# dselivanov/rsparse

Hardware: AMD Instinct MI355X
Metric: als_iterations_per_sec (higher is better)
Workload: dtype f32 (Gram products of rows > 512 / <= 32 non-zeros as 2 x fp16 / 3 x bf16 split terms of the fp32 operands, fp32 accumulate; everything else fp32); 1 GPU; WRMF implicit ALS, CG(3), synthetic 10000000x1000000, 500155883 nnz, rank 128, lambda 0.1; survey_config=3, feedback=implicit, n_items=1000000, nnz=500155883, rank=128, solver=conjugate_gradient, cg_steps=3, parallelism=rows sharded x1, factors replicated

## Files before the change

rsparse_amd/csrc/wrmf_capi.cpp:

```cpp
#include "../../include/rsparse_wrmf_hip.h"

#include <cxxabi.h>

#include <algorithm>
#include <cfloat>
#include <cmath>
#include <cstdio>
#include <cstdlib>
#include <cstring>
#include <string>
#include <vector>

#include "wrmf_capi_common.h"
#include "wrmf_topk_plan.h"

using namespace rsparse_hip;

struct rsparse_hip_csc {
  DevCSC d;
  int device = 0;
  std::vector<void*> owned;
};

namespace {
// ... 180 lines not shown
  return implicit || solver != RSPARSE_SOLVER_CHOLESKY || lambda != 0.0;
}

int check_variant(unsigned solver, int with_biases, double global_bias, bool implicit = true) {
  if (solver > RSPARSE_SOLVER_NNLS) return fail(RSPARSE_HIP_ERR_INVALID, "unknown solver code");
  if (with_biases && implicit && solver == RSPARSE_SOLVER_CONJUGATE_GRADIENT)
    return fail(RSPARSE_HIP_ERR_UNSUPPORTED, "with_user_item_bias + conjugate_gradient with implicit feedback is not on the device path");
  (void)global_bias;
  return RSPARSE_HIP_OK;
}

struct BiasTerms {
  const float* rhs_vals;
  const float* loss_tgt;
  const float* rhs_init;
  float tgt_const = 1.f;
  float gbias = 0.f;
};

hipError_t take_value_stats(const DevCSC& d, const float* d_X, int64_t nx, hipStream_t s, const float* d_absmax) {
  if (d.vals_frozen && !d.vstats && hipMalloc(&d.vstats, 2 * sizeof(unsigned)) != hipSuccess) d.vstats = nullptr;
  if (d.vals_frozen && d.vstats && d.vstats_valid && d.vstats_stream == s)
    return launch_ne_stats(d_X, nx, d.vals, d.nnz, g_ws.ne_stats, s, d_absmax, d.vstats, nullptr);
  hipError_t e = launch_ne_stats(d_X, nx, d.vals, d.nnz, g_ws.ne_stats, s, d_absmax, nullptr,
                                 (d.vals_frozen && d.vstats) ? d.vstats : nullptr);
  if (e == hipSuccess && d.vals_frozen && d.vstats) { d.vstats_valid = true; d.vstats_stream = s; }
  return e;
}

int run_half_iteration(const rsparse_hip_csc* conf, bool implicit, const float* d_X, float* d_Y,
                       const float* d_XtX, int rank, double lambda, unsigned solver, unsigned cg_steps,
                       int dynamic_lambda, double* d_loss_rows_out, hipStream_t s, const BiasTerms* bias = nullptr,
                       const float* d_absmax = nullptr) {
  if (!conf) return fail(RSPARSE_HIP_ERR_INVALID, "conf is NULL");
  if (!d_X || !d_Y) return fail(RSPARSE_HIP_ERR_INVALID, "X or Y is NULL");
  if (implicit && !d_XtX) return fail(RSPARSE_HIP_ERR_INVALID, "XtX is NULL");
  if (rank <= 0) return fail(RSPARSE_HIP_ERR_INVALID, "rank must be positive");
  if (rank > RSPARSE_HIP_MAX_RANK) return fail(RSPARSE_HIP_ERR_UNSUPPORTED, "rank > 256 is not on the device path");
  int rc = check_variant(solver, 0, 0.0);
  if (rc) return rc;
  if ((rc = g_ws.ensure_device())) return rc;
  const DevCSC& d = conf->d;
  const bool pad_to_128 = solver == RSPARSE_SOLVER_CHOLESKY && !bias && rank > 64 && rank < 128 && zero_padding_is_neutral(implicit, solver, lambda);
  const bool pad_to_64 = solver == RSPARSE_SOLVER_CHOLESKY && !bias && rank < 64 && zero_padding_is_neutral(implicit, solver, lambda);
  if (((rank % 4 != 0 && rank < 128) || pad_to_128 || pad_to_64) && zero_padding_is_neutral(implicit, solver, lambda)) {
    const int kp = pad_to_128 ? 128 : (pad_to_64 ? 64 : ((rank + 3) & ~3));
    const size_t nx = (size_t)d.n_rows * kp, ny = (size_t)d.n_cols * kp, ng = (size_t)kp * kp;
    HIP_TRY(g_ws.pad_buf.ensure(nx + ny + ng + 256 + 16));
    float* Xp = g_ws.pad_buf;
// ... 140 lines not shown
    if (implicit) {
      a.ne_stats = g_ws.ne_stats;
      a.mf_XtX = d_XtX;
      if (rank != 128) {
        HIP_TRY(g_ws.mf_G.ensure((size_t)128 * 128));
        hipError_t pe = launch_pad_gramian(d_XtX, rank, 128, g_ws.mf_G, s);
        if (pe != hipSuccess) return hip_fail(pe, "launch_pad_gramian");
        a.mf_XtX = g_ws.mf_G;
      }
    }
  }
  if (!a.ne_stats && (cgq || ne_chol) && implicit && (qs.ne.wg > 0 || qs.mf_n > 0) && ne_supported(rank) && (!bias || gb_cg)) {
    if ((rc = want_stats())) return rc;
    a.ne_stats = g_ws.ne_stats;
    if (gb_cg && cgq) {
      const int n_ne = d.q_off[1];
      HIP_TRY(g_ws.gb_r0.ensure((size_t)n_ne * rank));
      HIP_TRY(g_ws.gb_slot.ensure((size_t)d.n_cols));
      hipError_t ge = launch_gb_row_terms(a, d.q_order, n_ne, g_ws.gb_r0, g_ws.gb_slot, s);
      if (ge != hipSuccess) return hip_fail(ge, "launch_gb_row_terms");
      a.ne_r0 = g_ws.gb_r0; a.ne_r0_slot = g_ws.gb_slot;
    }
  }
  if (cgq && !ne_supported(rank) && d.q_stream_off && d.q_nnz[0] > 0 && cg_steps >= 1 && cg_steps <= 4) {
    HIP_TRY(g_ws.tscr.ensure((size_t)(cg_steps + 1) * (size_t)d.q_nnz[0]));
    a.tscr = g_ws.tscr;
  }
  if (!cg && solver == RSPARSE_SOLVER_CHOLESKY && d.q_order && d.q_n_lr > 0 && chol_lr_supported(a, implicit)) {
    HIP_TRY(g_ws.lr_M.ensure((size_t)3 * 128 * 128));
    if ((rc = want_stats())) return rc;
    a.lr_rows = d.q_order + d.q_lr_first; a.n_lr = d.q_n_lr; a.lr_flags = g_ws.ne_stats + 2; a.lr_M = g_ws.lr_M;
    a.lr_n_gt32 = d.q_gt32 - d.q_lr_first; a.lr_n_gt16 = d.q_pair_first - d.q_lr_first;
    a.lr_n_gt48 = d.q_gt48 - d.q_lr_first;
  }
  const bool chol = !cg && solver == RSPARSE_SOLVER_CHOLESKY;
  if (chol && d.q_order && d.q_n_lr > 0 && chol_lrx_supported(a, implicit)) {
    if ((rc = want_stats())) return rc;
    a.wave_stats = g_ws.ne_stats;
    a.lr_rows = d.q_order + d.q_lr_first; a.n_lr = d.q_n_lr; a.lrx = 1;
    a.lr_n_gt32 = d.q_gt32 - d.q_lr_first; a.lr_n_gt16 = d.q_pair_first - d.q_lr_first;
    a.lr_n_gt48 = d.q_gt48 - d.q_lr_first;
  }
  if (chol && chol_wave_supported(rank) && padded_rank(rank) == 64) {
    if ((rc = want_stats())) return rc;
    a.wave_stats = g_ws.ne_stats;
  }
// ... 42 lines not shown
  if (rank < 2) return fail(RSPARSE_HIP_ERR_INVALID, "with_biases needs rank >= 2 (a row of ones and a bias row)");
  if (rank > RSPARSE_HIP_MAX_RANK) return fail(RSPARSE_HIP_ERR_UNSUPPORTED, "rank > 256 is not on the device path");
  int rc = g_ws.ensure_device();
  if (rc) return rc;
  const DevCSC& d = conf->d;
  const int k1 = rank - 1;
  const int xoff = is_x_bias_last_row ? 0 : 1;
  const int xb = is_x_bias_last_row ? rank - 1 : 0;
  const int ioff = is_x_bias_last_row ? 1 : 0;
  const int ooff = is_x_bias_last_row ? 0 : 1;
  const int k1p = zero_padding_is_neutral(false, solver, lambda) ? std::min((k1 + 3) & ~3, RSPARSE_HIP_MAX_RANK) : k1;
  const size_t nx = (size_t)d.n_rows * k1p, ny = (size_t)d.n_cols * k1p, nv = (size_t)std::max<int64_t>(d.nnz, 1);
  HIP_TRY(g_ws.bias_buf.ensure(nx + ny + nv + 16));
  float* Xp = g_ws.bias_buf;
  float* Yp = Xp + nx;
  float* vp = Yp + ny;
  hipError_t e;
  if ((e = launch_pad_rows(d_X, rank, xoff, k1, k1p, d.n_rows, Xp, s)) != hipSuccess) return hip_fail(e, "launch_pad_rows");
  if ((e = launch_pad_rows(d_Y, rank, ioff, k1, k1p, d.n_cols, Yp, s)) != hipSuccess) return hip_fail(e, "launch_pad_rows");
  e = launch_bias_shift_values(d.vals, d.row_idx, d_X, rank, xb, d.nnz, vp, s);
  if (e != hipSuccess) return hip_fail(e, "launch_bias_shift_values");
  rsparse_hip_csc shifted;
  shifted.d = conf->d; shifted.device = conf->device;
  shifted.d.vals_frozen = false; shifted.d.vstats_valid = false; shifted.d.vstats = nullptr;
  shifted.d.vals = vp;
  rc = run_half_iteration(&shifted, false, Xp, Yp, nullptr, k1p, lambda, solver, cg_steps, dynamic_lambda,
                          d_loss_rows_out, s);
  if (rc) return rc;
  if (d.n_cols > 0)
    HIP_TRY(hipMemcpy2DAsync(d_Y + ooff, (size_t)rank * 4, Yp, (size_t)k1p * 4, (size_t)k1 * 4, (size_t)d.n_cols,
                             hipMemcpyDeviceToDevice, s));
  return RSPARSE_HIP_OK;
}

int run_half_iteration_implicit_biased(const rsparse_hip_csc* conf, const float* d_X, float* d_Y, const float* d_XtX,
                                       int rank, double lambda, unsigned solver, int is_x_bias_last_row,
                                       double* d_loss_rows_out, hipStream_t s, double global_bias = 0.0,
                                       bool dbl_threshold = false) {
  if (!conf) return fail(RSPARSE_HIP_ERR_INVALID, "conf is NULL");
  if (!d_X || !d_Y || !d_XtX) return fail(RSPARSE_HIP_ERR_INVALID, "X, Y or XtX is NULL");
  if (rank < 2) return fail(RSPARSE_HIP_ERR_INVALID, "with_biases needs rank >= 2 (a row of ones and a bias row)");
  if (rank > RSPARSE_HIP_MAX_RANK) return fail(RSPARSE_HIP_ERR_UNSUPPORTED, "rank > 256 is not on the device path");
  int rc = g_ws.ensure_device();
  if (rc) return rc;
  const DevCSC& d = conf->d;
  const int k1 = rank - 1;
  const int xoff = is_x_bias_last_row ? 0 : 1, xb = is_x_bias_last_row ? rank - 1 : 0;
// ... 219 lines not shown
}

int rsparse_hip_values_to_float_device(int64_t n, const double* d_src, float* d_dst, void* stream) {
  if (n < 0) return fail(RSPARSE_HIP_ERR_INVALID, "negative length");
  if (n > 0 && (!d_src || !d_dst)) return fail(RSPARSE_HIP_ERR_INVALID, "NULL array");
  if (n == 0) return RSPARSE_HIP_OK;
  hipError_t e = launch_f64_to_f32(d_src, d_dst, (size_t)n, static_cast<hipStream_t>(stream));
  if (e != hipSuccess) return hip_fail(e, "launch_f64_to_f32");
  return RSPARSE_HIP_OK;
}

int rsparse_hip_csc_destroy(rsparse_hip_csc* m) {
  if (!m) return RSPARSE_HIP_OK;
  for (void* p : m->owned) (void)hipFree(p);
  if (m->d.vstats) (void)hipFree(m->d.vstats);
  delete m;
  return RSPARSE_HIP_OK;
}

int rsparse_hip_csc_freeze_values(rsparse_hip_csc* m, int frozen) {
  if (!m) return fail(RSPARSE_HIP_ERR_INVALID, "NULL handle");
  m->d.vals_frozen = frozen != 0;
  m->d.vstats_valid = false;
  return RSPARSE_HIP_OK;
}

int rsparse_hip_csc_info(const rsparse_hip_csc* m, int64_t info_out[40]) {
  if (!m || !info_out) return fail(RSPARSE_HIP_ERR_INVALID, "NULL argument");
  for (int b = 0; b < 40; b++) info_out[b] = 0;
  for (int b = 0; b < 6; b++) {
    info_out[8 + b] = m->d.q_off[b + 1] - m->d.q_off[b];
    info_out[14 + b] = m->d.q_nnz[b];
  }
  info_out[20] = m->d.q_cfg;
  info_out[21] = m->d.q_ne.nseg;
  for (int b = 0; b < 6; b++) {
    info_out[22 + b] = cgq_bucket_wpr(m->d.q_cfg, b);
    info_out[28 + b] = cgq_bucket_capq(m->d.q_cfg, b);
    info_out[34 + b] = cgq_bucket_waves(m->d.q_cfg, b) * (cgq_bucket_stream(m->d.q_cfg, b) ? -1 : 1);
  }
  info_out[0] = m->d.n_rows; info_out[1] = m->d.n_cols; info_out[2] = m->d.nnz;
  info_out[3] = m->d.n_long; info_out[4] = m->d.max_len; info_out[5] = m->d.nnz_long;
  info_out[6] = m->d.n_empty; info_out[7] = m->d.short_max;
  return RSPARSE_HIP_OK;
}

// ... 909 lines not shown
```

rsparse_amd/csrc/wrmf_cg_mf.hip:

```cpp
#include <cstdio>
#include <utility>

#pragma clang diagnostic ignored "-Winline-asm"

#include "wrmf_internal.h"
#include "wrmf_device.h"

namespace rsparse_hip {
namespace {
using namespace dev;
constexpr int MF_A0 = 0;
#define MF_TOP "a255"
}
}

#include "wrmf_mf.h"

namespace rsparse_hip {
namespace {

__device__ __forceinline__ void cgm_operands_hi(const float (&x)[16], f16x8& h0, f16x8& h1) {
  float b0[8], b1[8];
#pragma unroll
  for (int e = 0; e < 8; e++) {
// ... 471 lines not shown
      for (int I = 0; I < 4; I++) {
        b[I] = sw.rhs[32 * I + n];
        x[I] = sw.x0[4 * n + I];
      }
    }
    auto rd_m1 = [&](auto tt, auto vt) { return mf_rd<16 * decltype(tt)::value + decltype(vt)::value>(); };
    auto g_tile = [&](auto tt, float (&g)[16]) {
      constexpr int T = decltype(tt)::value;
#pragma unroll
      for (int q = 0; q < 4; q++) {
        const float4 t = sm.G[T][ln][q];
        g[4 * q] = t.x; g[4 * q + 1] = t.y; g[4 * q + 2] = t.z; g[4 * q + 3] = t.w;
      }
    };
    float r[4], p[4], ap[4];
    cgm_matvec(rd_m1, g_tile, sw, un_m1, n, hf, ln, x, ap);
#pragma unroll
    for (int I = 0; I < 4; I++) { r[I] = b[I] - ap[I]; p[I] = r[I]; }
    double rsold = (double)cgm_dot(r, r, hf);
    for (int stp = 0; stp < a.cg_steps; stp++) {
      cgm_matvec(rd_m1, g_tile, sw, un_m1, n, hf, ln, p, ap);
      const float alpha = (float)(rsold / (double)cgm_dot(p, ap, hf));
#pragma unroll
      for (int I = 0; I < 4; I++) { x[I] = fmaf(alpha, p[I], x[I]); r[I] = fmaf(-alpha, ap[I], r[I]); }
      const double rsnew = (double)cgm_dot(r, r, hf);
      if (rsnew < (double)kCgTol) break;
      const float beta = (float)(rsnew / rsold);
#pragma unroll
      for (int I = 0; I < 4; I++) p[I] = fmaf(p[I], beta, r[I]);
      rsold = rsnew;
    }
    if (hf == 0) {
      int row2 = row;
      asm volatile("" : "+s"(row2));
      float* yr = a.Y + (size_t)row2 * k;
      *reinterpret_cast<float4*>(yr + 4 * n) = make_float4(x[0], x[1], x[2], x[3]);
    }
    auto rd_m2 = [&](auto tt, auto vt) {
      constexpr int T = decltype(tt)::value, v = decltype(vt)::value;
      if constexpr (T < 6) return mf_rd<160 + 16 * T + v>();
      else return hi[T - 6][v];
    };
    float yMy;
    {
      wave_sync();
      if (hf == 0) {
#pragma unroll
// ... 30 lines not shown
    wave_sync();
  }
  if (lane == 0) a.loss_partials[loss_slot0 + 4 * blockIdx.x + wv] = sw.loss;
}

}
}

#define CGM_KERNEL(NAME, SYM)                                                                                                     \
  extern "C" __global__ __launch_bounds__(256, 1) __attribute__((amdgpu_num_vgpr(128))) void NAME(                                  \
      rsparse_hip::AlsArgs a, const int32_t* __restrict__ rows, int n_rows, int loss_slot0) {                                       \
    rsparse_hip::als_cg_mf_body<SYM>(a, rows, n_rows, loss_slot0);                                                                  \
  }
CGM_KERNEL(rsparse_hip_als_cg_mf_implicit, true)
CGM_KERNEL(rsparse_hip_als_cg_mf_implicit_any, false)
#undef CGM_KERNEL

namespace rsparse_hip {

bool cg_mf_supported(int k, bool implicit) { return implicit && k == 128; }
int cg_mf_grid(int n_rows) { return std::max(1, std::min((n_rows + 3) / 4, kCgMfGrid)); }
int cg_mf_loss_slots(int n_rows) { return 2 * 4 * cg_mf_grid(n_rows); }

hipError_t launch_als_cg_mf(const AlsArgs& a, const int32_t* rows, int n_rows, int loss_slot0, hipStream_t s, hipEvent_t* ev_slot) {
  if (n_rows <= 0) return hipSuccess;
  if (!a.ne_stats || !cg_mf_supported(a.k, true) || (reinterpret_cast<uintptr_t>(a.X) & 3)) return hipErrorInvalidValue;
  const int grid = cg_mf_grid(n_rows);
  auto kern = rsparse_hip_als_cg_mf_implicit;
  auto kern2 = rsparse_hip_als_cg_mf_implicit_any;
  const int b1 = (int)sizeof(CgmSmem<12>), b2 = (int)sizeof(CgmSmem<20>);
  hipError_t e;
  if ((e = hipFuncSetAttribute(reinterpret_cast<const void*>(kern), hipFuncAttributeMaxDynamicSharedMemorySize, b1)) != hipSuccess) return e;
  if ((e = hipFuncSetAttribute(reinterpret_cast<const void*>(kern2), hipFuncAttributeMaxDynamicSharedMemorySize, b2)) != hipSuccess) return e;
  prof_note(ev_slot, reinterpret_cast<const void*>(kern));
  hipLaunchKernelGGL(kern, dim3(grid), dim3(256), b1, s, a, rows, n_rows, loss_slot0);
  hipLaunchKernelGGL(kern2, dim3(grid), dim3(256), b2, s, a, rows, n_rows, loss_slot0 + 4 * grid);
  return hipGetLastError();
}

}
```

rsparse_amd/csrc/wrmf_cgp.hip:

```cpp
#include "wrmf_internal.h"
#include "wrmf_device.h"

namespace rsparse_hip {
namespace {

using namespace dev;

constexpr int kPairMaxSweeps = 4;

template <int NQ, bool QUAD = false>
struct PairSmem {
  static constexpr int KP = 128, ps = KP + 8, os = QUAD ? KP + 8 : KP + 4;
  static constexpr int cols = QUAD ? 16 : 8;
  static constexpr int pcs = QUAD ? 2 * ps : ps;
  static constexpr size_t gfrag = NQ == 16 ? (size_t)4 * 16 * 1024 : 0;
  static constexpr size_t nxt = NQ == 16 ? (size_t)4 * 2 * 2 * 64 * 4 : 0;
  static constexpr size_t pub = (size_t)2 * cols * ps * 2, out = (size_t)cols * os * 4;
  static_assert(!QUAD || (pub == out && (size_t)pcs * 2 == (size_t)os * 4), "QUAD: one column, one stretch of LDS");
  static constexpr size_t bytes = gfrag + (QUAD ? pub : pub + out) + (size_t)4 * 8 * NQ * 4 + nxt + 16;
};
static_assert(PairSmem<16>::bytes <= 81920 && PairSmem<16, true>::bytes <= 81920, "two workgroups per CU");

template <bool GB, bool KFULL = false, int NQ = 8, bool QUAD = false>
__global__ __launch_bounds__(256, 2) void als_cgp_kernel(AlsArgs a, const int32_t* __restrict__ rows, int n_rows, int iters,
// ... 387 lines not shown
    auto dot16 = [&](const float(&u)[RPN], const float(&w)[RPN]) {
      float s = 0.f;
#pragma unroll
      for (int rr = 0; rr < RPN; rr++) s = fmaf(u[rr], w[rr], s);
      return row16_sum(s);
    };

    float dummy = 0.f;
    sweep(x, 0, r, dummy);
    if constexpr (KFULL)
      request_indices(it + 1 < iters && ridx(it + 1) < n_rows, p1_c, p2_c - p1_c, (it + 1) & 1);
#pragma unroll
    for (int rr = 0; rr < RPN; rr++) p[rr] = r[rr];
    float rsold = dot16(r, r);
    bool conv = !live;
    for (int itc = 0; itc < a.cg_steps; ++itc) {
      sweep(p, 1, ap, dummy);
      const float pap = dot16(p, ap);
      const float alpha = conv ? 0.f : (float)((double)rsold / (double)pap);
      wave_sync();
      if (lgrp) tacc[lslot] = fmaf(alpha, tcur[lslot], tacc[lslot]);
      wave_sync();
#pragma unroll
      for (int rr = 0; rr < RPN; rr++) {
        x[rr] = fmaf(alpha, p[rr], x[rr]);
        r[rr] = fmaf(-alpha, ap[rr], r[rr]);
      }
      const float rsnew = dot16(r, r);
      if (!conv) {
        if (rsnew < kCgTol) {
          conv = true;
        } else {
          const float beta = (float)((double)rsnew / (double)rsold);
#pragma unroll
          for (int rr = 0; rr < RPN; rr++) p[rr] = fmaf(p[rr], beta, r[rr]);
          rsold = rsnew;
        }
      }
    }
    float rl = 0.f;
    sweep(x, 2, ap, rl);
    if constexpr (KFULL) {
      settle_indices();
    }
    if (live) {
      const float xx = dot16(x, x);
      wloss += (double)rl + a.lambda_loss * (double)xx;
      if (QUAD || g2 == 0) {
#pragma unroll
        for (int b = 0; b < NV; b++) {
          const int off = b * 16 * VW + i * VW;
          if (off < k) {
            float4 pc;
            float* pf = reinterpret_cast<float*>(&pc);
#pragma unroll
            for (int c = 0; c < VW; c++) pf[c] = x[b * VW + c];
            *reinterpret_cast<float4*>(yrow + off) = pc;
          }
        }
// ... 49 lines not shown
```

rsparse_amd/csrc/wrmf_cgq.hip:

```cpp
#include <algorithm>

#include "wrmf_internal.h"
#include "wrmf_device.h"

namespace rsparse_hip {
namespace {

using namespace dev;

constexpr int kGvFirstMinCapq = 16;
constexpr int kStreamPrefixQ = 4;
constexpr int kIdxPrefetchMaxWpr = 2;

constexpr int kMaxSavedSweeps = 4;

template <int KP>
struct QG {
  static constexpr int RPN = KP / 16;
  static constexpr int VW = RPN >= 4 ? 4 : RPN;
  static constexpr int NV = RPN / VW;
  __device__ static __forceinline__ int elem(int i, int r) { return (r / VW) * (16 * VW) + i * VW + (r % VW); }
};

template <int VW>
// ... 796 lines not shown
          if (s2 == itc) alph[s2] = alpha;
        if constexpr (TSAVE) {
          wave_sync();
          const int ln = opaque_lane<WIDEQ>(lane);
#pragma unroll
          for (int s2 = 0; s2 < NSL; s2++) {
            const int sl = NSL == 1 ? (lane & (CAP - 1)) : ln + 64 * s2;
            if (CAP % 64 == 0 || sl < CAP) tacc[sl] = fmaf(alpha, tcur[sl], tacc[sl]);
          }
          wave_sync();
        }
        if constexpr (CVLDS) {
          if (g == 0) {
#pragma unroll
            for (int b = 0; b < NV; b++) {
              piece_t pc = *x_piece(b);
              float* pf = reinterpret_cast<float*>(&pc);
#pragma unroll
              for (int c = 0; c < VW; c++) pf[c] = fmaf(alpha, p[b * VW + c], pf[c]);
              *x_piece(b) = pc;
            }
          }
        }
#pragma unroll
        for (int rr = 0; rr < RPN; rr++) {
          if constexpr (!CVLDS) x[rr] = fmaf(alpha, p[rr], x[rr]);
          r[rr] = fmaf(-alpha, ap[rr], r[rr]);
        }
        const float rsnew = dot16(r, r);
        if (rsnew < kCgTol) {
          conv = true;
        } else {
          const float beta = (float)((double)rsnew / (double)rsold);
#pragma unroll
          for (int rr = 0; rr < RPN; rr++) p[rr] = fmaf(p[rr], beta, r[rr]);
          rsold = rsnew;
        }
      }
    }
    if constexpr (CVLDS) {
      wave_sync();
#pragma unroll
      for (int b = 0; b < NV; b++) {
        const piece_t pc = *x_piece(b);
        const float* pf = reinterpret_cast<const float*>(&pc);
#pragma unroll
        for (int c = 0; c < VW; c++) x[b * VW + c] = pf[c];
      }
    }
    float rl = 0.f;
    sweep(x, 2, ap, rl, live);
    if constexpr (META_LATE) p1_c = rfl(p1_c), p2_c = rfl(p2_c);
    if constexpr (DMAPF) wait_vm<0>();
    if constexpr (IDXPF && STREAM == 0) {
      asm volatile("" : "+v"(pf_id), "+v"(pf_c));
    }
    if (live && tw == 0) {
      const float xx = dot16(x, x);
      const double wl_row = IMPLICIT ? (double)rl + a.lambda_loss * (double)xx : (double)(rl + lam_use * xx);
// ... 135 lines not shown
            forked = true;                                                                                  \
          }                                                                                                 \
          bs = g_bs.st[B];                                                                                  \
          if ((err = hipStreamWaitEvent(bs, g_bs.fork, 0)) != hipSuccess) return err;                       \
        }                                                                                                   \
        if (D.stream && ne_supported(a.k)) {                                                                \
           \
           \
           \
           \
          const bool mside = overlap && q.ne.wg > 0 && q.mf_n > 0;                                          \
           \
          if (mside && (err = hipEventRecord(g_bs.fork0, s)) != hipSuccess) return err;                     \
          if (q.ne.wg > 0 &&                                                                                \
              (err = launch_als_ne(a, q, IMPLICIT, a.loss_partials + slot, bs, q.mf_n > 0 ? nullptr : (ev ? ev + B : nullptr))) != hipSuccess) \
            return err;                                                                                     \
          if (q.mf_n > 0) {                                                                                 \
            hipStream_t ms = bs;                                                                            \
            if (mside) {                                                                                    \
              ms = g_bs.st[B];                                                                              \
              if ((err = hipStreamWaitEvent(ms, g_bs.fork0, 0)) != hipSuccess) return err;                  \
            }                                                                                               \
            if ((err = launch_als_cg_mf(a, q.mf_rows, q.mf_n, (int)(slot + (size_t)(q.ne.entries + q.ne.nsplit)), ms, \
                                        ev ? ev + B : nullptr)) != hipSuccess)                              \
              return err;                                                                                   \
            if (mside) {                                                                                    \
              if ((err = hipEventRecord(g_bs.done[B], ms)) != hipSuccess) return err;                       \
              if ((err = hipStreamWaitEvent(s, g_bs.done[B], 0)) != hipSuccess) return err;                 \
            }                                                                                               \
          }                                                                                                 \
        } else if constexpr (D.stream && KP > 32) {        \
          return hipErrorInvalidValue;                                                                      \
        } else if constexpr (B == 1 && team4_split(KP, GB)) {                                              \
           \
           \
          const int first = q.off[B], wide = team4_wide_first(q), split = team4_first(q);                   \
          const int n_main = wide - first, n_w4 = split - wide, n_t4 = q.off[B + 1] - split;                \
          const int g_main = cgq_bucket_grid(n_main, B, CFG), g_w4 = cgq_team4_wide_grid(n_w4);             \
          if ((err = launch_bucket<KP, D.waves, D.capq, D.wpr, D.stream, IMPLICIT, GB>(a, q.order + first, n_main, g_main, slot, \
                                                                                  bs, ev ? ev + B : nullptr)) != hipSuccess) \
            return err;                                                                                     \
          if ((err = launch_bucket<KP, kTeam4Waves, kTeam4WideCapq, kTeam4Waves, 0, IMPLICIT, GB>(          \
                   a, q.order + wide, n_w4, g_w4, slot + (size_t)g_main * D.waves, bs,                      \
                   n_main > 0 ? nullptr : (ev ? ev + B : nullptr))) != hipSuccess)                          \
            return err;                                                                                     \
          if ((err = launch_bucket<KP, kTeam4Waves, kTeam4Capq, kTeam4Waves, 0, IMPLICIT, GB>(              \
                   a, q.order + split, n_t4, cgq_team4_grid(n_t4),                                          \
// ... 109 lines not shown
```

rsparse_amd/csrc/wrmf_internal.h:

```cpp
#pragma once
#include <hip/hip_runtime.h>
#include <cstdint>
#include <string>

#include "wrmf_schedule.h"

namespace rsparse_hip {

constexpr float kCgTol = 1e-10f;
constexpr double kCgTolD = 1e-10;
constexpr int kScdMaxIter = 10000;
constexpr float kScdTol = 1e-4f;
constexpr double kScdTolD = 1e-4;
constexpr float kNnlsEps = 1e-16f;
constexpr double kNnlsEpsD = 1e-16;

struct NeListSet {
  const int32_t* rows = nullptr;
  const int32_t* ptr = nullptr;
  int wg = 0;
  int entries = 0;
  const int32_t* segs = nullptr;
  int nseg = 0;
  const int32_t* split_rows = nullptr;
// ... 13 lines not shown
  int max_len = 0;
  const int32_t* q_order = nullptr;
  int q_off[7] = {0, 0, 0, 0, 0, 0, 0};
  int q_cfg = 0;
  int q_pair_first = 0;
  int q_team4_first = 0;
  int q_team4_wide_first = 0;
  int64_t q_nnz[6] = {0, 0, 0, 0, 0, 0};
  const int64_t* q_stream_off = nullptr;
  int q_n_chol_long = 0;
  int q_gt32 = 0;
  int q_gt48 = 0;
  int q_lr_first = 0, q_n_lr = 0;
  NeListSet q_ne;
  NeListSet q_ne1;
  int q_n_nec = 0;
  NeListSet q_nec;
  int64_t nnz_long = 0;
  int n_empty = 0;
  mutable bool vals_frozen = false;
  mutable bool vstats_valid = false;
  mutable unsigned* vstats = nullptr;
  mutable hipStream_t vstats_stream = nullptr;
};

struct AlsArgs {
  const int32_t* col_ptrs;
  const int32_t* row_idx;
  const float* vals;
  const float* X;
  float* Y;
  const float* XtX;
  const int32_t* long_rows;
  int n_long;
  int n_cols;
  int k;
  int cg_steps;
  float lambda;
  double lambda_loss;
  int dynamic_lambda;
  double* loss_partials;
  int* fail_counter;
  int* fail_rows;
  int fail_cap;
  const float* zero_row;
  const float* rhs_vals;
// ... 21 lines not shown
  float* lr_M;
  const int32_t* ne_segs;
  float* ne_seg_scratch;
  int* ne_seg_flags;
  int ne_chol;
  int ne_chol_min;
  const unsigned* ne_stats;
  const float* mf_XtX;
  const unsigned* wave_stats;
};

struct QSchedule {
  const int32_t* order;
  int off[7];
  int pair_first;
  int team4_first;
  int team4_wide_first;
  bool pair_wide;
  bool pair_quad = false;
  int cfg;
  NeListSet ne;
  const int32_t* mf_rows = nullptr;
  int mf_n = 0;
};
int cgq_default_cfg();
void cgq_set_launch_mode(int mode);
int cgq_num_buckets();
int cgq_bucket_wpr(int cfg, int b);
int cgq_bucket_capq(int cfg, int b);
int cgq_bucket_waves(int cfg, int b);
int cgq_bucket_stream(int cfg, int b);
int cgq_bucket_grid(int n_rows, int bucket, int cfg);
int cgq_team4_grid(int n_rows);
int cgq_team4_wide_grid(int n_rows);
int cgq_bucket_of(int len, int cfg);
size_t cgq_loss_slots(const QSchedule& q, int k, bool implicit);
bool cgp_supported(int k, bool implicit);
bool cgp_wide_supported(int k, bool implicit, bool gbias);
bool cgp_quad_supported(int k, bool implicit, bool gbias);
enum CgpForm { kCgpPair = 0, kCgpWide = 1, kCgpQuad = 2 };
inline int cgp_rows_per_wave(CgpForm form) { return form == kCgpQuad ? 4 : 2; }
hipError_t launch_als_cgp(const AlsArgs& a, const int32_t* rows, int n_rows, CgpForm form, size_t loss_slot0, hipStream_t s,
                          hipEvent_t* ev_slot);
bool ne_supported(int k);
constexpr int kNeMinLen = 512;
constexpr int kNeSegFloats = 4 * (11 * 16 * 64 + 128 + 2);
// ... 18 lines not shown
constexpr int kCholLongGrid = 512;
constexpr int kCholLrGrid = 65536;
size_t chol2_loss_slots(int n_cols);
bool chol_lr_supported(const AlsArgs& a, bool implicit);
bool chol_lrx_supported(const AlsArgs& a, bool implicit);
hipError_t launch_als_chol_lrx(const AlsArgs& a, const int32_t* rows, int n_rows, const unsigned* stats, int loss_slot0,
                               hipStream_t s, hipEvent_t* ev_slot);
hipError_t launch_als_chol_lr(const AlsArgs& a, const int32_t* rows, int n_rows, float* M, float* Mt, unsigned* flags,
                              int loss_slot0, hipStream_t s, hipEvent_t* ev_slot = nullptr);
hipError_t launch_als_chol2(const AlsArgs& a, bool implicit, hipStream_t s, hipEvent_t* ev = nullptr);
bool chol_wave_supported(int k);
hipError_t launch_als_chol_wave(const AlsArgs& a, bool implicit, int grid, int loss_slot0, hipStream_t s, hipEvent_t* ev_slot);
constexpr int kCholMfMax = 512;
constexpr int kCholMfGrid = 256 * 32;
bool chol_mf_supported(int k);
int chol_mf_grid(int n_rows);
int chol_mf_loss_slots(int n_rows, bool implicit);
hipError_t launch_als_chol_mf(const AlsArgs& a, bool implicit, const int32_t* rows, int n_rows, int loss_slot0, hipStream_t s,
                              hipEvent_t* ev_slot);
constexpr int kCgMfGrid = 256 * 16;
bool cg_mf_supported(int k, bool implicit);
int cg_mf_grid(int n_rows);
int cg_mf_loss_slots(int n_rows);
hipError_t launch_als_cg_mf(const AlsArgs& a, const int32_t* rows, int n_rows, int loss_slot0, hipStream_t s, hipEvent_t* ev_slot);
hipError_t launch_als_nnls(const AlsArgs& a, bool implicit, hipStream_t s, hipEvent_t* ev = nullptr);
constexpr int kLuGrid = 64;
constexpr int kFailCap = 1 << 16;
hipError_t launch_als_lu_fallback(const AlsArgs& a, bool implicit, size_t loss_slot0, hipStream_t s);
hipError_t launch_fail_roll(int* fails, hipStream_t s);
constexpr int kSumStageBlocks = 256;
hipError_t launch_sum_partials(const double* partials, size_t n, double* out, hipStream_t s, double* tail = nullptr);
hipError_t launch_bias_shift_values(const float* vals, const int32_t* row_idx, const float* X, int k, int bias_row,
                                    int64_t nnz, float* out, hipStream_t s);
hipError_t launch_bias_sweep(const int32_t* p, const int32_t* i, const float* x, const float* other, int n_cols,
                             float lambda, int dynamic_lambda, int non_negative, float* out, hipStream_t s);
hipError_t launch_values_sum(const float* x, int64_t n, double* partials, double* out, hipStream_t s);
hipError_t launch_bias_implicit_terms(const float* vals, const int32_t* row_idx, const float* X, int k, int bias_row,
                                      int64_t nnz, float global_bias, float* rhs_vals, float* loss_tgt, hipStream_t s);
hipError_t launch_bias_rhs_init(const float* X, int k, int off, int k1, int bias_row, float global_bias, int n,
                                float* scratch, float* out, hipStream_t s);
size_t bias_rhs_init_scratch_floats();
hipError_t launch_pad_rows(const float* src, int src_stride, int src_off, int k1, int k1p, int64_t n, float* dst, hipStream_t s);
hipError_t launch_pad_gramian(const float* G, int k1, int k1p, float* Gp, hipStream_t s);
hipError_t launch_bias_implicit_prep(const int32_t* p, const float* x, int n_cols, int n_other, double lambda,
                                     double* means, double* adj, hipStream_t s);
hipError_t launch_bias_implicit_sweep(const int32_t* p, const int32_t* i, const float* x, const float* other, int n_cols,
                                      int n_other, const double* other_sum, const double* means, const double* adj,
// ... 239 lines not shown
```

rsparse_amd/csrc/wrmf_kernels.hip:

```cpp
#include "wrmf_internal.h"
#include "wrmf_device.h"

namespace rsparse_hip {
namespace {

using namespace dev;

template <int KP, int T, int W, bool IMPLICIT>
struct CgSmem {
  static constexpr int LDT = Geo<KP>::LDT;
  static constexpr size_t gram_floats = IMPLICIT ? (size_t)KP * KP : 0;
  static constexpr size_t tile_floats = (size_t)W * T * LDT;
  static constexpr size_t vec_floats = (size_t)W * KP;
  static constexpr size_t red_floats = (size_t)2 * W * KP + 2 * W;
  static constexpr size_t short_bytes = (gram_floats + tile_floats + vec_floats) * 4 + 16;
  static constexpr size_t long_bytes = (gram_floats + tile_floats + vec_floats + red_floats) * 4 + 16;
};

template <int KP, int W>
__device__ __forceinline__ void load_gram_lds(float* sG, const float* __restrict__ G, int k, int tid) {
  for (int e = tid; e < KP * KP; e += W * 64) {
    const int r = e / KP, c = e % KP;
    sG[e] = (r < k && c < k) ? G[(size_t)r * k + c] : 0.f;
  }
// ... 75 lines not shown
    for (int u = 0; u < EPL; u++) { p[u] = r[u]; rs = fmaf(r[u], r[u], rs); }
    float rsold = wave_sum(rs);

    for (int it = 0; it < a.cg_steps; ++it) {
      wave_sync();
      put_vec<KP>(vec, p, lane, active);
      wave_sync();
      t = tile_dot<KP, T>(tile, vec, lane);
      wgt = jvalid ? (IMPLICIT ? (c - 1.f) * t : t) : 0.f;
#pragma unroll
      for (int u = 0; u < EPL; u++) ap[u] = 0.f;
      tile_axpy<KP>(tile, wgt, cnt, lane, active, ap);
      if constexpr (IMPLICIT) {
        gram_mv<KP>(sG, vec, 0, KP, lane, active, 1.f, ap);
      } else {
#pragma unroll
        for (int u = 0; u < EPL; u++) ap[u] = fmaf(lam_use, p[u], ap[u]);
      }
      float pap = 0.f;
#pragma unroll
      for (int u = 0; u < EPL; u++) pap = fmaf(p[u], ap[u], pap);
      pap = wave_sum(pap);
      const float alpha = (float)((double)rsold / (double)pap);
      rs = 0.f;
#pragma unroll
      for (int u = 0; u < EPL; u++) {
        x[u] = fmaf(alpha, p[u], x[u]);
        r[u] = fmaf(-alpha, ap[u], r[u]);
        rs = fmaf(r[u], r[u], rs);
      }
      const float rsnew = wave_sum(rs);
      if (rsnew < kCgTol) break;
      const float beta = (float)((double)rsnew / (double)rsold);
#pragma unroll
      for (int u = 0; u < EPL; u++) p[u] = fmaf(p[u], beta, r[u]);
      rsold = rsnew;
    }

    wave_sync();
    put_vec<KP>(vec, x, lane, active);
    wave_sync();
    t = tile_dot<KP, T>(tile, vec, lane);
    const float d = IMPLICIT ? ltgt - t : c - t;
    const float lj = (jvalid && lane < T) ? (IMPLICIT ? c * d * d : d * d) : 0.f;
    const float rl = wave_sum(lj);
    float xx = 0.f;
#pragma unroll
    for (int u = 0; u < EPL; u++) xx = fmaf(x[u], x[u], xx);
    xx = wave_sum(xx);
    wloss += IMPLICIT ? (double)rl + a.lambda_loss * (double)xx : (double)(rl + lam_use * xx);
// ... 123 lines not shown
#pragma unroll
          for (int u = 0; u < EPL; u++) out[u] = fmaf(mode == 0 ? -lam_use : lam_use, v[u], out[u]);
        } else if (gb && mode == 0) {
#pragma unroll
          for (int u = 0; u < EPL; u++) out[u] += (active && e0 + u < k) ? a.rhs_init[e0 + u] : 0.f;
        }
      }
      buf ^= 1;
    };

    float dummy = 0.f;
    sweep(x, 0, r, dummy);
    float rs = 0.f;
#pragma unroll
    for (int u = 0; u < EPL; u++) { p[u] = r[u]; rs = fmaf(r[u], r[u], rs); }
    float rsold = wave_sum(rs);
    for (int it = 0; it < a.cg_steps; ++it) {
      sweep(p, 1, ap, dummy);
      float pap = 0.f;
#pragma unroll
      for (int u = 0; u < EPL; u++) pap = fmaf(p[u], ap[u], pap);
      pap = wave_sum(pap);
      const float alpha = (float)((double)rsold / (double)pap);
      rs = 0.f;
#pragma unroll
      for (int u = 0; u < EPL; u++) {
        x[u] = fmaf(alpha, p[u], x[u]);
        r[u] = fmaf(-alpha, ap[u], r[u]);
        rs = fmaf(r[u], r[u], rs);
      }
      const float rsnew = wave_sum(rs);
      if (rsnew < kCgTol) break;
      const float beta = (float)((double)rsnew / (double)rsold);
#pragma unroll
      for (int u = 0; u < EPL; u++) p[u] = fmaf(p[u], beta, r[u]);
      rsold = rsnew;
    }
    float rl = 0.f;
    sweep(x, 2, ap, rl);
    float xx = 0.f;
#pragma unroll
    for (int u = 0; u < EPL; u++) xx = fmaf(x[u], x[u], xx);
    xx = wave_sum(xx);
    if (wv == 0) {
      wloss += IMPLICIT ? (double)rl + a.lambda_loss * (double)xx : (double)(rl + lam_use * xx);
#pragma unroll
      for (int u = 0; u < EPL; u++)
        if (active && e0 + u < k) yrow[e0 + u] = x[u];
    }
  }
// ... 316 lines not shown
```

rsparse_amd/csrc/wrmf_ne.hip:

```cpp
#include <type_traits>
#include <utility>

#include "wrmf_internal.h"
#include "wrmf_device.h"
#include "wrmf_ldlt.h"

namespace rsparse_hip {
namespace {

using namespace dev;

constexpr int kStepNnz = 16;

struct NeMfmaOp { int slot, m, R, C, pa, pb; };
struct NeUnit { int kind, t, pair; };

template <int KP, int NS, bool IMPLICIT, bool SYM = false, bool QUAD = false>
struct NeRoles {
  static_assert(!SYM || (IMPLICIT && NS == 2), "SYM: implicit feedback, two fp16 terms");
  static_assert(!QUAD || (SYM && KP == 128), "QUAD: the fp16 path at rank 128");
  static constexpr int NB = KP / 32;
  static constexpr int NT = NB * (NB + 1) / 2;
  static constexpr bool PAIR = IMPLICIT && KP == 128 && !QUAD;
  static constexpr int NROLES = QUAD ? 4 : (PAIR ? 2 : 1);
// ... 930 lines not shown
    } else {
    float r[NB], p[NB], ap[NB];
#pragma unroll
    for (int t = 0; t < NB; t++) p[t] = x[t];
    float r0x[NB];
#pragma unroll
    for (int t = 0; t < NB; t++) r0x[t] = 0.f;
    if constexpr (GB) {
      const int sl = sload(a.ne_r0_slot + row);
#pragma unroll
      for (int t = 0; t < NB; t++) r0x[t] = (32 * t + d < k) ? a.ne_r0[(size_t)sl * k + 32 * t + d] : 0.f;
    }
    double rsold = 0.0;
    bool conv = false;
    for (int it = 0; it <= a.cg_steps; ++it) {
      matvec(p, ap);
      if (it == 0) {
#pragma unroll
        for (int t = 0; t < NB; t++) p[t] = r[t] = (b[t] - ap[t]) + r0x[t];
        rsold = (double)dot(r, r);
      } else if (!conv) {
        const float alpha = (float)(rsold / (double)dot(p, ap));
#pragma unroll
        for (int t = 0; t < NB; t++) {
          x[t] = fmaf(alpha, p[t], x[t]);
          r[t] = fmaf(-alpha, ap[t], r[t]);
        }
        const double rsnew = (double)dot(r, r);
        if (rsnew < (double)kCgTol) {
          conv = true;
        } else {
          const float beta = (float)(rsnew / rsold);
#pragma unroll
          for (int t = 0; t < NB; t++) p[t] = fmaf(p[t], beta, r[t]);
          rsold = rsnew;
        }
      }
    }
    }

    wave_sync();
    if (h == 0) {
#pragma unroll
      for (int t = 0; t < NB; t++) pub[32 * t + d] = x[t];
    }
    wave_sync();
    float qf = 0.f;
    with_role([&](auto rc) { qf = quad_form(rc, pub, x); });
    if (lane == 0) sScal[16 + wv] = qf;
    const float yb = dot(x, b), yy = dot(x, x);
    __syncthreads();
    if (wv == 0) {
      const double q = ((double)sScal[16] + (double)sScal[17]) + ((double)sScal[18] + (double)sScal[19]);
      const double tau = GB ? (double)a.loss_tgt_const : 1.0;
      const double fit = tau * tau * sc_row - 2.0 * tau * (double)yb + q;
      const double reg = IMPLICIT ? a.lambda_loss * (double)yy : (double)(lam_use * yy);
      if (lane == 0) {
        sYloss[nbuf] = row_bad ? 0.0 : fit + reg;
// ... 215 lines not shown
```

rsparse_amd/csrc/wrmf_wide_cg.hip:

```cpp
#include <algorithm>

#include "wrmf_internal.h"
#include "wrmf_device.h"

namespace rsparse_hip {
namespace {

using namespace dev;

template <int EPL>
struct WVec {
  float c[EPL];
};

struct WideCgArgs {
  const int32_t* col_ptrs;
  const int32_t* row_idx;
  const float* vals;
  const float* X;
  float* Y;
  const float* XtX;
  int n_cols, k, cg_steps, dynamic_lambda, n_hi;
  double lambda_loss;
  double* loss_partials;
// ... 150 lines not shown
    const float lam_use = IMPLICIT ? (float)a.lambda_loss : (float)(a.lambda_loss * (a.dynamic_lambda ? (double)n : 1.0));
    Vec x, r, pv;
#pragma unroll
    for (int e = 0; e < EPL; e++) x.c[e] = lk[e] ? yrow[lane + 64 * e] : 0.f;
    {
      const Vec t0 = wide_row_pass<EPL, IMPLICIT, 0, TEAM>(a, k, p1, n, x, lk, lc, lane, wv, sT);
      Vec g0;
      if constexpr (IMPLICIT) g0 = gmv(x);
#pragma unroll
      for (int e = 0; e < EPL; e++) r.c[e] = t0.c[e] - (IMPLICIT ? g0.c[e] : lam_use * x.c[e]);
    }
    pv = r;
    double rsold = (double)dot(r, r);
    for (int it = 0; it < a.cg_steps; it++) {
      Vec ap = wide_row_pass<EPL, IMPLICIT, 1, TEAM>(a, k, p1, n, pv, lk, lc, lane, wv, sT);
      {
        Vec g1;
        if constexpr (IMPLICIT) g1 = gmv(pv);
#pragma unroll
        for (int e = 0; e < EPL; e++) ap.c[e] += IMPLICIT ? g1.c[e] : lam_use * pv.c[e];
      }
      const float alpha = (float)(rsold / (double)dot(pv, ap));
#pragma unroll
      for (int e = 0; e < EPL; e++) {
        x.c[e] = fmaf(alpha, pv.c[e], x.c[e]);
        r.c[e] = fmaf(-alpha, ap.c[e], r.c[e]);
      }
      const double rsnew = (double)dot(r, r);
      if (rsnew < (double)kCgTol) break;
      const float beta = (float)(rsnew / rsold);
#pragma unroll
      for (int e = 0; e < EPL; e++) pv.c[e] = fmaf(pv.c[e], beta, r.c[e]);
      rsold = rsnew;
    }
    if (TEAM == 1 || wv == 0) {
#pragma unroll
      for (int e = 0; e < EPL; e++)
        if (lane + 64 * e < k) yrow[lane + 64 * e] = x.c[e];
    }
    const Vec lrow = wide_row_pass<EPL, IMPLICIT, 2, TEAM>(a, k, p1, n, x, lk, lc, lane, wv, sT);
    const float xx = dot(x, x);
    wloss += IMPLICIT ? (double)lrow.c[0] + a.lambda_loss * (double)xx : (double)(lrow.c[0] + lam_use * xx);
  }
  if constexpr (TEAM > 1) {
    if (tid == 0) a.loss_partials[slot0 + blockIdx.x] = wloss;
  } else {
    if (lane == 0) sLoss[wv] = wloss;
    __syncthreads();
    if (tid == 0) a.loss_partials[slot0 + blockIdx.x] = (sLoss[0] + sLoss[1]) + (sLoss[2] + sLoss[3]);
  }
// ... 49 lines not shown
```

Baseline: 8.819 iterations/s.

## Skip final CG residual update and launch only the live cg_mf kernel variant

Across the CG kernels, the last iteration now stops after updating x and skips the residual update, its norm and the p update, since nothing uses them afterwards. Some template variants are excluded via constexpr flags. Separately, after value stats are computed for frozen values, one stats word is read back to the host once. That flag selects which of the two cg_mf kernels is needed, and the unneeded one is skipped with its loss slots zeroed. The trade is a one-time host sync when stats are taken, plus added branching in the kernels.

After: 8.835 iterations/s, median of 5. No clear change (+0.2%).

```diff
diff --git a/rsparse_amd/csrc/wrmf_capi.cpp b/rsparse_amd/csrc/wrmf_capi.cpp
--- a/rsparse_amd/csrc/wrmf_capi.cpp
+++ b/rsparse_amd/csrc/wrmf_capi.cpp
@@ -226,9 +226,16 @@
   if (d.vals_frozen && !d.vstats && hipMalloc(&d.vstats, 2 * sizeof(unsigned)) != hipSuccess) d.vstats = nullptr;
   if (d.vals_frozen && d.vstats && d.vstats_valid && d.vstats_stream == s)
     return launch_ne_stats(d_X, nx, d.vals, d.nnz, g_ws.ne_stats, s, d_absmax, d.vstats, nullptr);
+  d.vstats_valid = false; d.vstats_lt1 = -1;
   hipError_t e = launch_ne_stats(d_X, nx, d.vals, d.nnz, g_ws.ne_stats, s, d_absmax, nullptr,
                                  (d.vals_frozen && d.vstats) ? d.vstats : nullptr);
-  if (e == hipSuccess && d.vals_frozen && d.vstats) { d.vstats_valid = true; d.vstats_stream = s; }
+  if (e == hipSuccess && d.vals_frozen && d.vstats) {
+    unsigned lt1 = 0;
+    if ((e = hipMemcpyAsync(&lt1, d.vstats + 1, sizeof(unsigned), hipMemcpyDeviceToHost, s)) != hipSuccess) return e;
+    if ((e = hipStreamSynchronize(s)) != hipSuccess) return e;
+    d.vstats_lt1 = lt1 != 0u ? 1 : 0;
+    d.vstats_valid = true; d.vstats_stream = s;
+  }
   return e;
 }
 
@@ -415,6 +422,7 @@
       a.ne_r0 = g_ws.gb_r0; a.ne_r0_slot = g_ws.gb_slot;
     }
   }
+  if (qs.mf_n > 0 && stats_taken && d.vals_frozen && d.vstats_valid) qs.mf_live = d.vstats_lt1;
   if (cgq && !ne_supported(rank) && d.q_stream_off && d.q_nnz[0] > 0 && cg_steps >= 1 && cg_steps <= 4) {
     HIP_TRY(g_ws.tscr.ensure((size_t)(cg_steps + 1) * (size_t)d.q_nnz[0]));
     a.tscr = g_ws.tscr;
@@ -503,7 +511,7 @@
   if (e != hipSuccess) return hip_fail(e, "launch_bias_shift_values");
   rsparse_hip_csc shifted;
   shifted.d = conf->d; shifted.device = conf->device;
-  shifted.d.vals_frozen = false; shifted.d.vstats_valid = false; shifted.d.vstats = nullptr;
+  shifted.d.vals_frozen = false; shifted.d.vstats_valid = false; shifted.d.vstats_lt1 = -1; shifted.d.vstats = nullptr;
   shifted.d.vals = vp;
   rc = run_half_iteration(&shifted, false, Xp, Yp, nullptr, k1p, lambda, solver, cg_steps, dynamic_lambda,
                           d_loss_rows_out, s);
@@ -769,6 +777,7 @@
   if (!m) return fail(RSPARSE_HIP_ERR_INVALID, "NULL handle");
   m->d.vals_frozen = frozen != 0;
   m->d.vstats_valid = false;
+  m->d.vstats_lt1 = -1;
   return RSPARSE_HIP_OK;
 }
 
diff --git a/rsparse_amd/csrc/wrmf_cg_mf.hip b/rsparse_amd/csrc/wrmf_cg_mf.hip
--- a/rsparse_amd/csrc/wrmf_cg_mf.hip
+++ b/rsparse_amd/csrc/wrmf_cg_mf.hip
@@ -517,7 +517,10 @@
       cgm_matvec(rd_m1, g_tile, sw, un_m1, n, hf, ln, p, ap);
       const float alpha = (float)(rsold / (double)cgm_dot(p, ap, hf));
 #pragma unroll
-      for (int I = 0; I < 4; I++) { x[I] = fmaf(alpha, p[I], x[I]); r[I] = fmaf(-alpha, ap[I], r[I]); }
+      for (int I = 0; I < 4; I++) x[I] = fmaf(alpha, p[I], x[I]);
+      if (stp + 1 == a.cg_steps) break;
+#pragma unroll
+      for (int I = 0; I < 4; I++) r[I] = fmaf(-alpha, ap[I], r[I]);
       const double rsnew = (double)cgm_dot(r, r, hf);
       if (rsnew < (double)kCgTol) break;
       const float beta = (float)(rsnew / rsold);
@@ -594,7 +597,8 @@
 int cg_mf_grid(int n_rows) { return std::max(1, std::min((n_rows + 3) / 4, kCgMfGrid)); }
 int cg_mf_loss_slots(int n_rows) { return 2 * 4 * cg_mf_grid(n_rows); }
 
-hipError_t launch_als_cg_mf(const AlsArgs& a, const int32_t* rows, int n_rows, int loss_slot0, hipStream_t s, hipEvent_t* ev_slot) {
+hipError_t launch_als_cg_mf(const AlsArgs& a, const int32_t* rows, int n_rows, int loss_slot0, hipStream_t s, hipEvent_t* ev_slot,
+                            int live) {
   if (n_rows <= 0) return hipSuccess;
   if (!a.ne_stats || !cg_mf_supported(a.k, true) || (reinterpret_cast<uintptr_t>(a.X) & 3)) return hipErrorInvalidValue;
   const int grid = cg_mf_grid(n_rows);
@@ -604,9 +608,13 @@
   hipError_t e;
   if ((e = hipFuncSetAttribute(reinterpret_cast<const void*>(kern), hipFuncAttributeMaxDynamicSharedMemorySize, b1)) != hipSuccess) return e;
   if ((e = hipFuncSetAttribute(reinterpret_cast<const void*>(kern2), hipFuncAttributeMaxDynamicSharedMemorySize, b2)) != hipSuccess) return e;
-  prof_note(ev_slot, reinterpret_cast<const void*>(kern));
-  hipLaunchKernelGGL(kern, dim3(grid), dim3(256), b1, s, a, rows, n_rows, loss_slot0);
-  hipLaunchKernelGGL(kern2, dim3(grid), dim3(256), b2, s, a, rows, n_rows, loss_slot0 + 4 * grid);
+  prof_note(ev_slot, reinterpret_cast<const void*>(live == 1 ? kern2 : kern));
+  if (live == 0 || live == 1) {
+    const int dead0 = loss_slot0 + (live == 0 ? 4 * grid : 0);
+    if ((e = hipMemsetAsync(a.loss_partials + dead0, 0, (size_t)4 * grid * sizeof(double), s)) != hipSuccess) return e;
+  }
+  if (live != 1) hipLaunchKernelGGL(kern, dim3(grid), dim3(256), b1, s, a, rows, n_rows, loss_slot0);
+  if (live != 0) hipLaunchKernelGGL(kern2, dim3(grid), dim3(256), b2, s, a, rows, n_rows, loss_slot0 + 4 * grid);
   return hipGetLastError();
 }
 
diff --git a/rsparse_amd/csrc/wrmf_cgp.hip b/rsparse_amd/csrc/wrmf_cgp.hip
--- a/rsparse_amd/csrc/wrmf_cgp.hip
+++ b/rsparse_amd/csrc/wrmf_cgp.hip
@@ -433,19 +433,20 @@
       if (lgrp) tacc[lslot] = fmaf(alpha, tcur[lslot], tacc[lslot]);
       wave_sync();
 #pragma unroll
-      for (int rr = 0; rr < RPN; rr++) {
-        x[rr] = fmaf(alpha, p[rr], x[rr]);
-        r[rr] = fmaf(-alpha, ap[rr], r[rr]);
-      }
-      const float rsnew = dot16(r, r);
-      if (!conv) {
-        if (rsnew < kCgTol) {
-          conv = true;
-        } else {
-          const float beta = (float)((double)rsnew / (double)rsold);
-#pragma unroll
-          for (int rr = 0; rr < RPN; rr++) p[rr] = fmaf(p[rr], beta, r[rr]);
-          rsold = rsnew;
+      for (int rr = 0; rr < RPN; rr++) x[rr] = fmaf(alpha, p[rr], x[rr]);
+      if (itc + 1 != a.cg_steps) {
+#pragma unroll
+        for (int rr = 0; rr < RPN; rr++) r[rr] = fmaf(-alpha, ap[rr], r[rr]);
+        const float rsnew = dot16(r, r);
+        if (!conv) {
+          if (rsnew < kCgTol) {
+            conv = true;
+          } else {
+            const float beta = (float)((double)rsnew / (double)rsold);
+#pragma unroll
+            for (int rr = 0; rr < RPN; rr++) p[rr] = fmaf(p[rr], beta, r[rr]);
+            rsold = rsnew;
+          }
         }
       }
     }
diff --git a/rsparse_amd/csrc/wrmf_cgq.hip b/rsparse_amd/csrc/wrmf_cgq.hip
--- a/rsparse_amd/csrc/wrmf_cgq.hip
+++ b/rsparse_amd/csrc/wrmf_cgq.hip
@@ -842,19 +842,24 @@
             }
           }
         }
-#pragma unroll
-        for (int rr = 0; rr < RPN; rr++) {
-          if constexpr (!CVLDS) x[rr] = fmaf(alpha, p[rr], x[rr]);
-          r[rr] = fmaf(-alpha, ap[rr], r[rr]);
-        }
-        const float rsnew = dot16(r, r);
-        if (rsnew < kCgTol) {
-          conv = true;
-        } else {
-          const float beta = (float)((double)rsnew / (double)rsold);
-#pragma unroll
-          for (int rr = 0; rr < RPN; rr++) p[rr] = fmaf(p[rr], beta, r[rr]);
-          rsold = rsnew;
+        if constexpr (!CVLDS) {
+#pragma unroll
+          for (int rr = 0; rr < RPN; rr++) x[rr] = fmaf(alpha, p[rr], x[rr]);
+        }
+        constexpr bool kCutLast = !(KP == 128 && WPR == 8 && GB && KFULL) && !(KP == 64 && CAPQ == 32 && WPR == 1 && IMPLICIT) &&
+                                  !(KP == 32 && WPR > 1 && WPR < 8 && !IMPLICIT && KFULL);
+        if (!kCutLast || itc + 1 != a.cg_steps) {
+#pragma unroll
+          for (int rr = 0; rr < RPN; rr++) r[rr] = fmaf(-alpha, ap[rr], r[rr]);
+          const float rsnew = dot16(r, r);
+          if (rsnew < kCgTol) {
+            conv = true;
+          } else {
+            const float beta = (float)((double)rsnew / (double)rsold);
+#pragma unroll
+            for (int rr = 0; rr < RPN; rr++) p[rr] = fmaf(p[rr], beta, r[rr]);
+            rsold = rsnew;
+          }
         }
       }
     }
@@ -1036,7 +1041,7 @@
               if ((err = hipStreamWaitEvent(ms, g_bs.fork0, 0)) != hipSuccess) return err;                  \
             }                                                                                               \
             if ((err = launch_als_cg_mf(a, q.mf_rows, q.mf_n, (int)(slot + (size_t)(q.ne.entries + q.ne.nsplit)), ms, \
-                                        ev ? ev + B : nullptr)) != hipSuccess)                              \
+                                        ev ? ev + B : nullptr, q.mf_live)) != hipSuccess)                   \
               return err;                                                                                   \
             if (mside) {                                                                                    \
               if ((err = hipEventRecord(g_bs.done[B], ms)) != hipSuccess) return err;                       \
diff --git a/rsparse_amd/csrc/wrmf_internal.h b/rsparse_amd/csrc/wrmf_internal.h
--- a/rsparse_amd/csrc/wrmf_internal.h
+++ b/rsparse_amd/csrc/wrmf_internal.h
@@ -59,6 +59,7 @@
   mutable bool vstats_valid = false;
   mutable unsigned* vstats = nullptr;
   mutable hipStream_t vstats_stream = nullptr;
+  mutable int vstats_lt1 = -1;
 };
 
 struct AlsArgs {
@@ -126,6 +127,7 @@
   NeListSet ne;
   const int32_t* mf_rows = nullptr;
   int mf_n = 0;
+  int mf_live = -1;
 };
 int cgq_default_cfg();
 void cgq_set_launch_mode(int mode);
@@ -190,7 +192,8 @@
 bool cg_mf_supported(int k, bool implicit);
 int cg_mf_grid(int n_rows);
 int cg_mf_loss_slots(int n_rows);
-hipError_t launch_als_cg_mf(const AlsArgs& a, const int32_t* rows, int n_rows, int loss_slot0, hipStream_t s, hipEvent_t* ev_slot);
+hipError_t launch_als_cg_mf(const AlsArgs& a, const int32_t* rows, int n_rows, int loss_slot0, hipStream_t s, hipEvent_t* ev_slot,
+                            int live = -1);
 hipError_t launch_als_nnls(const AlsArgs& a, bool implicit, hipStream_t s, hipEvent_t* ev = nullptr);
 constexpr int kLuGrid = 64;
 constexpr int kFailCap = 1 << 16;
diff --git a/rsparse_amd/csrc/wrmf_kernels.hip b/rsparse_amd/csrc/wrmf_kernels.hip
--- a/rsparse_amd/csrc/wrmf_kernels.hip
+++ b/rsparse_amd/csrc/wrmf_kernels.hip
@@ -121,10 +121,13 @@
       for (int u = 0; u < EPL; u++) pap = fmaf(p[u], ap[u], pap);
       pap = wave_sum(pap);
       const float alpha = (float)((double)rsold / (double)pap);
+#pragma unroll
+      for (int u = 0; u < EPL; u++) x[u] = fmaf(alpha, p[u], x[u]);
+      constexpr bool kCutLast = !(KP == 128 && IMPLICIT) && !(KP == 32 && IMPLICIT && !VEC) && !(KP == 64 && !IMPLICIT && !VEC);
+      if (kCutLast && it + 1 == a.cg_steps) break;
       rs = 0.f;
 #pragma unroll
       for (int u = 0; u < EPL; u++) {
-        x[u] = fmaf(alpha, p[u], x[u]);
         r[u] = fmaf(-alpha, ap[u], r[u]);
         rs = fmaf(r[u], r[u], rs);
       }
@@ -294,10 +297,12 @@
       for (int u = 0; u < EPL; u++) pap = fmaf(p[u], ap[u], pap);
       pap = wave_sum(pap);
       const float alpha = (float)((double)rsold / (double)pap);
+#pragma unroll
+      for (int u = 0; u < EPL; u++) x[u] = fmaf(alpha, p[u], x[u]);
+      if (it + 1 == a.cg_steps) break;
       rs = 0.f;
 #pragma unroll
       for (int u = 0; u < EPL; u++) {
-        x[u] = fmaf(alpha, p[u], x[u]);
         r[u] = fmaf(-alpha, ap[u], r[u]);
         rs = fmaf(r[u], r[u], rs);
       }
diff --git a/rsparse_amd/csrc/wrmf_ne.hip b/rsparse_amd/csrc/wrmf_ne.hip
--- a/rsparse_amd/csrc/wrmf_ne.hip
+++ b/rsparse_amd/csrc/wrmf_ne.hip
@@ -976,18 +976,19 @@
       } else if (!conv) {
         const float alpha = (float)(rsold / (double)dot(p, ap));
 #pragma unroll
-        for (int t = 0; t < NB; t++) {
-          x[t] = fmaf(alpha, p[t], x[t]);
-          r[t] = fmaf(-alpha, ap[t], r[t]);
-        }
-        const double rsnew = (double)dot(r, r);
-        if (rsnew < (double)kCgTol) {
-          conv = true;
-        } else {
-          const float beta = (float)(rsnew / rsold);
-#pragma unroll
-          for (int t = 0; t < NB; t++) p[t] = fmaf(p[t], beta, r[t]);
-          rsold = rsnew;
+        for (int t = 0; t < NB; t++) x[t] = fmaf(alpha, p[t], x[t]);
+        if (KP == 64 || it != a.cg_steps) {
+#pragma unroll
+          for (int t = 0; t < NB; t++) r[t] = fmaf(-alpha, ap[t], r[t]);
+          const double rsnew = (double)dot(r, r);
+          if (rsnew < (double)kCgTol) {
+            conv = true;
+          } else {
+            const float beta = (float)(rsnew / rsold);
+#pragma unroll
+            for (int t = 0; t < NB; t++) p[t] = fmaf(p[t], beta, r[t]);
+            rsold = rsnew;
+          }
         }
       }
     }
diff --git a/rsparse_amd/csrc/wrmf_wide_cg.hip b/rsparse_amd/csrc/wrmf_wide_cg.hip
--- a/rsparse_amd/csrc/wrmf_wide_cg.hip
+++ b/rsparse_amd/csrc/wrmf_wide_cg.hip
@@ -196,10 +196,11 @@
       }
       const float alpha = (float)(rsold / (double)dot(pv, ap));
 #pragma unroll
-      for (int e = 0; e < EPL; e++) {
-        x.c[e] = fmaf(alpha, pv.c[e], x.c[e]);
-        r.c[e] = fmaf(-alpha, ap.c[e], r.c[e]);
-      }
+      for (int e = 0; e < EPL; e++) x.c[e] = fmaf(alpha, pv.c[e], x.c[e]);
+      constexpr bool kCutLast = !(IMPLICIT && TEAM == 1 && EPL >= 3);
+      if (kCutLast && it + 1 == a.cg_steps) break;
+#pragma unroll
+      for (int e = 0; e < EPL; e++) r.c[e] = fmaf(-alpha, ap.c[e], r.c[e]);
       const double rsnew = (double)dot(r, r);
       if (rsnew < (double)kCgTol) break;
       const float beta = (float)(rsnew / rsold);
```
